# dkohlsdorf/audio_pattern_discovery

Measured on AMD Instinct MI355X. Metric: DTW cell-updates/sec (whole node), higher is better.
Workload: dtype f32

## Files before the change

audio_pattern_discovery_amd/csrc/dtw_systolic.h:

```cpp
#pragma once
#include <type_traits>

#ifndef APD_ABLATE
#define APD_ABLATE 0
#endif

#include "dtw_common.h"

namespace apd {

typedef float apd_f32x4 __attribute__((ext_vector_type(4)));
constexpr uint32_t kNoFrame = 0xFFFFFF00u;

template <int D>
__device__ __forceinline__ void load_frame(float (&dst)[D], __amdgpu_buffer_rsrc_t rsrc, uint32_t byte_off)
{
    constexpr int DP4 = (D + 3) / 4;
#pragma unroll
    for (int q = 0; q < DP4; ++q) {
        const apd_f32x4 t = __builtin_bit_cast(apd_f32x4, __builtin_amdgcn_raw_buffer_load_b128(rsrc, byte_off + 16u * q, 0, 0));
        if (4 * q + 0 < D) dst[4 * q + 0] = t.x;
        if (4 * q + 1 < D) dst[4 * q + 1] = t.y;
        if (4 * q + 2 < D) dst[4 * q + 2] = t.z;
        if (4 * q + 3 < D) dst[4 * q + 3] = t.w;
    }
}

template <int D>
__device__ __forceinline__ void load_frame_dwords(float (&dst)[D], __amdgpu_buffer_rsrc_t rsrc, uint32_t byte_off)
{
#pragma unroll
    for (int k = 0; k < D; ++k)
        dst[k] = __builtin_bit_cast(float, __builtin_amdgcn_raw_buffer_load_b32(rsrc, byte_off + 4u * k, 0, 0));
}

template <int D, int DN>
__device__ __forceinline__ float frame_dist(const float (&x)[DN], const float (&y)[DN])
{
    float t = x[0] - y[0];
    float acc = t * t;
#pragma unroll
    for (int k = 1; k < D; ++k) {
        t = x[k] - y[k];
        acc = __builtin_fmaf(t, t, acc);
    }
    if (APD_ABLATE & 1) return acc;
    return __builtin_amdgcn_sqrtf(acc);
}

template <int D, int DN>
__device__ __forceinline__ float frame_sq_strict(const float (&x)[DN], const float (&y)[DN])
{
    float t = x[0] - y[0];
    float acc = t * t;
#pragma unroll
    for (int k = 1; k < D; ++k) {
        t = x[k] - y[k];
        const float sq = t * t;
        acc = acc + sq;
    }
    return acc;
}
template <int D, int DN>
__device__ __forceinline__ float frame_dist_strict(const float (&x)[DN], const float (&y)[DN])
{
    return __builtin_sqrtf(frame_sq_strict<D, DN>(x, y));
}

template <int D>
__device__ __forceinline__ float frame_sq_expanded_pre(const float (&xm)[D + 1], const float (&y)[D + 1])
{
    float acc = xm[D] + y[D];
#pragma unroll
    for (int k = 0; k < D; ++k) acc = __builtin_fmaf(xm[k], y[k], acc);
    return acc;
}
template <int D>
__device__ __forceinline__ void prescale_row_piece(apd_f32x4 &v, int piece)
{
    const bool np = piece == D / 4;
    v.x = (np && D % 4 == 0) ? v.x : -2.0f * v.x;
    v.y = (np && D % 4 == 1) ? v.y : -2.0f * v.y;
    v.z = (np && D % 4 == 2) ? v.z : -2.0f * v.z;
    v.w = (np && D % 4 == 3) ? v.w : -2.0f * v.w;
}
template <int D>
__device__ __forceinline__ float frame_sq_exact_pre(const float (&xm)[D + 1], const float (&y)[D + 1])
{
    float t = __builtin_fmaf(-0.5f, xm[0], -y[0]);
    float acc = t * t;
#pragma unroll
    for (int k = 1; k < D; ++k) {
        t = __builtin_fmaf(-0.5f, xm[k], -y[k]);
        acc = __builtin_fmaf(t, t, acc);
    }
    return acc;
}
template <int C, int G, bool UNIFORM_PEN>
__device__ __forceinline__ void dp_rows_step(float (&prev1)[C], float (&prev2)[C], const float (&d)[C], const bool (&g1)[C],
                                             const bool (&g2)[C], float del, float ins, float mat, int gl)
{
    float left1 = group_from_lower_wrap<G>(prev1[C - 1], APD_INF, gl);
    float left2 = group_from_lower_wrap<G>(prev2[C - 1], APD_INF, gl);
    float upr1 = APD_INF, upr2 = APD_INF;
#pragma unroll
    for (int c = 0; c < C; ++c) {
        if (APD_ABLATE & 2) { prev1[c] += d[c]; prev2[c] -= d[c]; continue; }
        const float up1 = (c < C - 1) ? prev1[(c + 1) % C] : upr1;
        const float up2 = (c < C - 1) ? prev2[(c + 1) % C] : upr2;
        const float r1 = select_node<UNIFORM_PEN>(left1, up1, prev1[c], d[c], del, ins, mat, (APD_ABLATE & 16) ? false : g1[c]);
        const float r2 = select_node<UNIFORM_PEN>(up2, left2, prev2[c], d[c], del, ins, mat, (APD_ABLATE & 16) ? false : g2[c]);
        prev1[c] = r1; prev2[c] = r2;
        left1 = r1; left2 = r2;
        if (c == 0) {
            upr1 = group_from_upper_wrap<G>(r1, APD_INF, gl);
            upr2 = group_from_upper_wrap<G>(r2, APD_INF, gl);
        }
    }
}
template <int C>
__device__ __forceinline__ void slow_phase_captures(float (&prev1)[C], float (&prev2)[C], float &res1, float &res2, int tau, int gl,
                                                    int tau_cap, int cw, int cstar)
{
    if (tau == gl) {
#pragma unroll
        for (int c = 0; c < C; ++c) if (c == cw) { prev1[c] = 0.0f; prev2[c] = 0.0f; }
    }
    if (tau == tau_cap) {
#pragma unroll
        for (int c = 0; c < C; ++c) if (c == cstar) { res1 = prev1[c]; res2 = prev2[c]; }
    }
}
template <int D, int C, int G, bool UNIFORM_PEN, bool HYBRID>
__global__ __launch_bounds__(256) void dtw_fused_systolic(const AlignLaunch L)
{
    static_assert(C >= 2 && (64 % G) == 0, "bad geometry");
    if (L.d_nonfinite != nullptr && *L.d_nonfinite != 0u) return;
    constexpr int DN = D + 1;
    constexpr int DP = (DN + 3) & ~3;
    constexpr int PPW = 64 / G;
    constexpr int WPT = kSlotsPerTile / (4 * PPW);
    const int lane = threadIdx.x & 63;
    const int gl = lane % G;
    const uint32_t xcd = blockIdx.x & 7u, q = blockIdx.x >> 3;
    const uint32_t tile = (q / WPT) * 8u + xcd;
    const uint32_t slot = ((q % WPT) * 4u + (threadIdx.x >> 6)) * PPW + lane / G;
    const PairInfo P = decode_pair_rows_b(L, tile, slot);
    const bool special = P.valid && (P.n == 1 || P.m == 1);
    const bool sweep = P.valid && !special;
    if (__ballot(sweep) == 0ull) {
        if (special && gl == 0) { const float s = (P.n == 1 && P.m == 1) ? 0.0f : APD_INF; store_pair(L, tile, P, s, s); }
        return;
    }
    const int n = sweep ? P.n : 1, m = sweep ? P.m : 1, w = sweep ? P.w : 2;
    const __amdgpu_buffer_rsrc_t rsrc = __builtin_amdgcn_make_buffer_rsrc((void *)L.d_frames, 0, L.frames_bytes, 0x00020000);
    const uint32_t a_off = (uint32_t)(P.A - L.d_frames) * 4u, b_off = (uint32_t)(P.B - L.d_frames) * 4u;
    constexpr uint32_t FB = DP * 4u;
    float ins = L.band.ins, del = L.band.del, mat = L.band.mat;
    float tau_thr = L.tau, nmax_b = P.nmax_b;
    asm volatile("" : "+v"(ins), "+v"(del), "+v"(mat), "+v"(tau_thr), "+v"(nmax_b));
    constexpr int R = (G == 64) ? 128 : 64;
    constexpr int LPF = DP / 4;
    constexpr int FPF = 64 / LPF;
    constexpr int RS = DP + 4;
    constexpr int U_ROWS = ((C + 1) % 2 == 0) ? (C + 1) : 2 * (C + 1);
    __shared__ float xring_all[4][(R + U_ROWS) * RS];
    float *const xring = xring_all[threadIdx.x >> 6];
    const int lead = __builtin_ctzll(__ballot(sweep));
    const uint32_t a_off_w = __builtin_amdgcn_readlane(a_off, lead);
    const int n_w = __builtin_amdgcn_readlane(n, lead);
    const int u0 = C * gl;
    const int two_w = 2 * w;

    bool g1[C], g2[C];
#pragma unroll
    for (int c = 0; c < C; ++c) {
        const int u = u0 + c;
        g1[c] = u >= two_w;
        g2[c] = (u == 0) | (u > two_w);
    }
    const int cw = w - u0;
    const int ustar = sweep_result_offset(n, m, w);
    const int cstar = ustar - u0;
    const int tau_cap = (n - 1) + gl;

    int w_bound = w;
    asm volatile("" : "+v"(w_bound));
    int my_total = sweep ? sweep_steps_needed(n, m, w_bound, C) : 0;
    int my_min = sweep ? (n - 1) : 0x7fffffff;
    int total = 0, min_rows = 0x7fffffff;
#pragma unroll
    for (int g = 0; g < PPW; ++g) {
        total = max(total, __builtin_amdgcn_readlane(my_total, g * G));
        min_rows = min(min_rows, __builtin_amdgcn_readlane(my_min, g * G));
    }
    constexpr int S = C + 1;
    constexpr int U = (S % 2 == 0) ? S : 2 * S;
    static_assert(U == U_ROWS, "ring copy sized for another unroll");
    constexpr bool MASKED_FETCH = HYBRID && (G == 32 || G == 8) && !(APD_ABLATE & 512);
    const int total_r = ((total + U - 1) / U) * U;
    int a_steps = G;
    if (UNIFORM_PEN && !HYBRID) {
        int w_max = 0;
#pragma unroll
        for (int g = 0; g < PPW; ++g) w_max = max(w_max, __builtin_amdgcn_readlane(w, g * G));
        a_steps = max(G, w_max + 1);
    }
    const int a_end = min(((a_steps + U - 1) / U) * U, total_r);
    const int b_end = min(max((min_rows / U) * U, a_end), total_r);

    float prev1[C], prev2[C];
#pragma unroll
    for (int c = 0; c < C; ++c) { prev1[c] = APD_INF; prev2[c] = APD_INF; }
    float res1 = 0.0f, res2 = 0.0f;

    float yf[S][DN];
#pragma unroll
    for (int c = 0; c < C; ++c) {
        const int j = u0 - gl + c - w;
        const int idx = (j >= 1) ? (min(j, m) - 1) : (HYBRID ? m : m + 1);
        load_frame<DN>(yf[c], rsrc, b_off + (uint32_t)idx * FB);
    }
#pragma unroll
    for (int k = 0; k < DN; ++k) yf[C][k] = 0.0f;
    if (HYBRID && !MASKED_FETCH && !(APD_ABLATE & 8)) {
        const int jt = 1 + (C - 1) * G - w;
        const uint32_t yo = b_off + (uint32_t)((jt >= 1) ? (min(jt, m) - 1) : m) * FB;
        load_frame<DN>(yf[C], rsrc, gl == G - 1 ? yo : kNoFrame);
    }
    constexpr int NFILL = (U + FPF - 1) / FPF;
    const int fill_f = lane / LPF, fill_q = lane % LPF;
    auto fill_load = [&](int first_row, apd_f32x4 (&regs)[NFILL]) __attribute__((always_inline)) {
#pragma unroll
        for (int f = 0; f < NFILL; ++f) {
            const int fi = f * FPF + fill_f;
            const bool act = (fill_f < FPF) & (fi < U);
            const uint32_t off = a_off_w + (uint32_t)(min(first_row + fi, n_w) - 1) * FB + 16u * fill_q;
            regs[f] = __builtin_bit_cast(apd_f32x4, __builtin_amdgcn_raw_buffer_load_b128(rsrc, act ? off : kNoFrame, 0, 0));
        }
    };
    auto fill_store = [&](int first_row, const apd_f32x4 (&regs)[NFILL]) __attribute__((always_inline)) {
#pragma unroll
        for (int f = 0; f < NFILL; ++f) {
            const int fi = f * FPF + fill_f;
            if ((fill_f < FPF) & (fi < U)) {
                apd_f32x4 v = regs[f];
                if (HYBRID) prescale_row_piece<D>(v, fill_q);
                const int slot = (first_row + fi) & (R - 1);
                *reinterpret_cast<apd_f32x4 *>(&xring[slot * RS + 4 * fill_q]) = v;
                if (slot < U) *reinterpret_cast<apd_f32x4 *>(&xring[(slot + R) * RS + 4 * fill_q]) = v;
            }
        }
    };
    for (int e = lane; e < G * DP; e += 64) {
        const int slot = (-(e / DP)) & (R - 1);
        const float v = HYBRID ? ((e % DP) == D ? APD_INF : 0.0f) : -APD_INF;
        xring[slot * RS + (e % DP)] = v;
        if (slot < U) xring[(slot + R) * RS + (e % DP)] = v;
    }
    {
        apd_f32x4 regs[NFILL];
        fill_load(1, regs);
        fill_store(1, regs);
    }
    asm volatile("" ::: "memory");
    auto read_row = [&](float (&dst)[DN], int row) __attribute__((always_inline)) {
        const float *p = &xring[(row & (R - 1)) * RS];
#pragma unroll
        for (int q = 0; q < LPF; ++q) {
            const apd_f32x4 t = *reinterpret_cast<const apd_f32x4 *>(p + 4 * q);
            if (4 * q + 0 < DN) dst[4 * q + 0] = t.x;
            if (4 * q + 1 < DN) dst[4 * q + 1] = t.y;
            if (4 * q + 2 < DN) dst[4 * q + 2] = t.z;
            if (4 * q + 3 < DN) dst[4 * q + 3] = t.w;
        }
    };
    auto read_row_at = [&](float (&dst)[DN], const float *p) __attribute__((always_inline)) {
#pragma unroll
        for (int q = 0; q < LPF; ++q) {
            const apd_f32x4 t = *reinterpret_cast<const apd_f32x4 *>(p + 4 * q);
            if (4 * q + 0 < DN) dst[4 * q + 0] = t.x;
            if (4 * q + 1 < DN) dst[4 * q + 1] = t.y;
            if (4 * q + 2 < DN) dst[4 * q + 2] = t.z;
            if (4 * q + 3 < DN) dst[4 * q + 3] = t.w;
        }
    };
    constexpr int NX = HYBRID ? 1 : 2;
    float xs[NX][DN];
    read_row(xs[0], 0 - gl);
#pragma unroll
    for (int k = 0; k < DN; ++k) xs[NX - 1][k] = (NX == 1) ? xs[0][k] : 0.0f;
    constexpr bool PIPE = (APD_ABLATE & 32) != 0;
    float dn[C];
#pragma unroll
    for (int c = 0; c < C; ++c) dn[c] = (PIPE && !HYBRID && c < C - 1) ? frame_dist_strict<D, DN>(xs[0], yf[c]) : 0.0f;

    auto advance_window = [&](int q) __attribute__((always_inline)) {
        const int r = q % S, e = (r + C) % S;
#pragma unroll
        for (int k = 0; k < (HYBRID ? DN : D); ++k) {
            if (APD_ABLATE & 4) { yf[e][k] = yf[(r + 1) % S][k] + yf[e][k]; continue; }
            yf[e][k] = MASKED_FETCH ? dpp_move<(G == 8) ? 0x101 : 0x130>(yf[(r + 1) % S][k], yf[e][k])
                                    : group_from_upper<G>(yf[(r + 1) % S][k], yf[e][k], gl);
        }
    };
    auto macro_steps = [&](int tau_begin, int tau_end, auto slow_tag) __attribute__((always_inline)) {
        constexpr bool SLOW = decltype(slow_tag)::value;
        uint32_t yo_cur = kNoFrame, yo_cap = kNoFrame, yo_step = 0u;
        if (!SLOW && gl == G - 1) {
            yo_cap = b_off + (uint32_t)(m - 1) * FB;
            yo_cur = min(b_off + (uint32_t)(tau_begin + ((HYBRID && !MASKED_FETCH) ? 1 : 0) + (C - 1) * G - w) * FB, yo_cap);
            yo_step = FB;
        }
        auto fetch_column = [&](float (&dst)[DN], int t) __attribute__((always_inline)) {
            if (APD_ABLATE & 8) return;
            if (SLOW) {
                const int jt = t + 1 + (C - 1) * G - w;
                const uint32_t yo = b_off + (uint32_t)((jt >= 1) ? (min(jt, m) - 1) : (HYBRID ? m : m + 1)) * FB;
                load_frame<DN>(dst, rsrc, gl == G - 1 ? yo : kNoFrame);
            } else {
                load_frame<DN>(dst, rsrc, yo_cur);
                yo_cur = min(yo_cur + yo_step, yo_cap);
            }
        };
        for (int tau0 = tau_begin; tau0 < tau_end; tau0 += U) {
            apd_f32x4 fill_regs[NFILL];
            fill_load(tau0 + U + 1, fill_regs);
            const float *const xrows = &xring[((tau0 + 1 - gl) & (R - 1)) * RS];
#pragma unroll
            for (int q = 0; q < U; ++q) {
                const int tau = tau0 + q;
                const int r = q % S;
                const int xa = HYBRID ? 0 : (q & 1), xb = HYBRID ? 0 : (xa ^ 1);
                const int e = (r + C) % S;
                if (!HYBRID) {
                    fetch_column(yf[e], tau);
                    read_row_at(xs[xb], xrows + q * RS);
                }
                float d[C];
                if (HYBRID) {
#pragma unroll
                    for (int c = 0; c < C; ++c) {
                        d[c] = frame_sq_expanded_pre<D>(xs[xa], yf[(r + c) % S]);
                    }
                    float dmin = d[0];
#pragma unroll
                    for (int c = 1; c + 1 < C; c += 2) dmin = __builtin_fminf(__builtin_fminf(dmin, d[c]), d[c + 1]);
                    if (C % 2 == 0) dmin = __builtin_fminf(dmin, d[C - 1]);
                    const bool any = (APD_ABLATE & 128) ? false : dmin < (xs[xa][D] + nmax_b) * tau_thr;
                    advance_window(q);
                    if (MASKED_FETCH) {
                        if (gl == G - 1) fetch_column(yf[e], tau);
                    }
                    if (__builtin_expect(__ballot(any) != 0ull, 0)) {
                        float nx = xs[xa][D];
                        asm volatile("" : "+v"(nx));
#pragma unroll
                        for (int c = 0; c < C; ++c) {
                            const float sc = nx + yf[(r + c) % S][D];
                            const float ex = frame_sq_exact_pre<D>(xs[xa], yf[(r + c) % S]);
                            d[c] = (d[c] < sc * tau_thr) ? ex : d[c];
                        }
                    }
                    if (!MASKED_FETCH) fetch_column(yf[r], tau + 1);
#pragma unroll
                    for (int c = 0; c < C; ++c) d[c] = (APD_ABLATE & 1) ? d[c] : __builtin_amdgcn_sqrtf(d[c]);
                    read_row_at(xs[0], xrows + q * RS);
                } else if (UNIFORM_PEN && !SLOW && !PIPE) {
                    float d2[C];
#pragma unroll
                    for (int c = 0; c < C; ++c) d2[c] = frame_sq_strict<D, DN>(xs[xa], yf[(r + c) % S]);
                    float dmin = d2[0];
#pragma unroll
                    for (int c = 1; c + 1 < C; c += 2) dmin = __builtin_fminf(__builtin_fminf(dmin, d2[c]), d2[c + 1]);
                    if (C % 2 == 0) dmin = __builtin_fminf(dmin, d2[C - 1]);
                    if (__builtin_expect(__ballot(!(dmin >= 0x1p-96f)) != 0ull, 0)) {
#pragma unroll
                        for (int c = 0; c < C; ++c) d[c] = __builtin_sqrtf(d2[c]);
                    } else {
#pragma unroll
                        for (int c = 0; c < C; ++c) d[c] = sqrt_rn_finite(d2[c]);
                    }
                } else {
#pragma unroll
                    for (int c = 0; c < C; ++c)
                        d[c] = (UNIFORM_PEN && PIPE && c < C - 1) ? dn[c] : frame_dist_strict<D, DN>(xs[xa], yf[(r + c) % S]);
                    if (PIPE) {
#pragma unroll
                        for (int c = 0; c < C - 1; ++c) dn[c] = frame_dist_strict<D, DN>(xs[xb], yf[(r + 1 + c) % S]);
                    }
                }
                dp_rows_step<C, G, UNIFORM_PEN>(prev1, prev2, d, g1, g2, del, ins, mat, gl);
                if (SLOW) slow_phase_captures<C>(prev1, prev2, res1, res2, tau, gl, tau_cap, cw, cstar);
                if (!HYBRID) advance_window(q);
            }
            fill_store(tau0 + U + 1, fill_regs);
            asm volatile("" ::: "memory");
        }
    };
    macro_steps(0, a_end, std::true_type{});
    macro_steps(a_end, b_end, std::false_type{});
    macro_steps(b_end, total_r, std::true_type{});

    if (P.valid && gl == (sweep ? ustar / C : 0)) {
        if (sweep) {
            const float denom = (float)(n + m);
            store_pair_rows_b(L, tile, P, res1 / denom, res2 / denom);
        } else {
            const float s = (P.n == 1 && P.m == 1) ? 0.0f : APD_INF;
            store_pair(L, tile, P, s, s);
        }
    }
}

typedef float apd_f32x2 __attribute__((ext_vector_type(2)));
template <int DN>
__device__ __forceinline__ void read_frame_lds(float (&dst)[DN], const float *p)
{
    constexpr int FULL = DN / 4, TAIL = DN % 4;
#pragma unroll
    for (int k = 0; k < FULL; ++k) {
        const apd_f32x4 t = *reinterpret_cast<const apd_f32x4 *>(p + 4 * k);
        dst[4 * k + 0] = t.x; dst[4 * k + 1] = t.y; dst[4 * k + 2] = t.z; dst[4 * k + 3] = t.w;
    }
    if (TAIL >= 2) {
        const apd_f32x2 t = *reinterpret_cast<const apd_f32x2 *>(p + 4 * FULL);
        dst[4 * FULL + 0] = t.x; dst[4 * FULL + 1] = t.y;
    }
    if (TAIL == 1) dst[4 * FULL] = p[4 * FULL];
    if (TAIL == 3) dst[4 * FULL + 2] = p[4 * FULL + 2];
}

constexpr int shared_column_ring_floats(int rc, int u, int dp) { return (((rc + u) * dp + ((rc + u + 7) / 8) * 4) * 4 + 255) / 256 * 64; }

template <int D, int C, int G>
__global__ __launch_bounds__(256) void dtw_fused_systolic_shared(const AlignLaunch L)
{
    static_assert(C >= 2 && G == 16, "one ring per wavefront: four lane groups");
    if (L.d_nonfinite != nullptr && *L.d_nonfinite != 0u) return;
    constexpr int DN = D + 1;
    constexpr int DP = (DN + 3) & ~3;
    constexpr int PPW = 64 / G;
    constexpr int WPT = kSlotsPerTile / (4 * PPW);
    constexpr int S = C + 1;
    constexpr int U = shared_column_unroll(C);
    constexpr int RC = shared_column_ring_frames(G, C);
    constexpr int R = 64;
    constexpr int LPF = DP / 4;
    constexpr int FPF = 64 / LPF;
    constexpr int RS = DP + 4;
    constexpr uint32_t FB = DP * 4u;
    constexpr int XRING = (R + U) * RS;
    constexpr int CRING = shared_column_ring_floats(RC, U, DP);
    static_assert(FPF >= U && RC % 8 == 0, "one wave-wide load per fill");
    static_assert(RC >= (G - 1) * (C - 1) + 2 * U + (int)shared_column_slack(KernelGeom{KernelGeom::SharedColumns, G, C}),
                  "ring too short for the spread of w the tile plan admits");
    extern __shared__ __attribute__((aligned(16))) float apd_shared_lds[];
    const int lane = threadIdx.x & 63, wave = threadIdx.x >> 6;
    const int gl = lane % G;
    float *const xring = apd_shared_lds + wave * XRING;
    float *const crings = apd_shared_lds + 4 * XRING;
    int *const wg_words = reinterpret_cast<int *>(crings + PPW * CRING);
    const uint32_t xcd = blockIdx.x & 7u, q = blockIdx.x >> 3;
    const uint32_t tile = (q / WPT) * 8u + xcd;
    const uint32_t sub = q % WPT;
    const uint32_t slot = ((sub % 4u) * 4u + wave) * kTile + (sub / 4u) * 4u + lane / G;
    const PairInfo P = decode_pair_rows_b(L, tile, slot);
    const bool special = P.valid && (P.n == 1 || P.m == 1);
    const bool sweep = P.valid && !special;
    const int n = sweep ? P.n : 1, m = sweep ? P.m : 1, w = sweep ? P.w : 2;
    const int u0 = C * gl;
    const int two_w = 2 * w;
    int w_bound = w;
    asm volatile("" : "+v"(w_bound));
    int my_total = sweep ? sweep_steps_needed(n, m, w_bound, C) : 0;
    int my_min = sweep ? (n - 1) : 0x7fffffff;
    int my_w = sweep ? w : 0x7fffffff;
    int total = 0, min_rows = 0x7fffffff, w_lo = 0x7fffffff;
#pragma unroll
    for (int g = 0; g < PPW; ++g) {
        total = max(total, __builtin_amdgcn_readlane(my_total, g * G));
        min_rows = min(min_rows, __builtin_amdgcn_readlane(my_min, g * G));
        w_lo = min(w_lo, __builtin_amdgcn_readlane(my_w, g * G));
    }
    if (lane == 0) { wg_words[2 * wave] = total; wg_words[2 * wave + 1] = w_lo; }
    __syncthreads();
    total = 0; w_lo = 0x7fffffff;
#pragma unroll
    for (int k = 0; k < 4; ++k) { total = max(total, wg_words[2 * k]); w_lo = min(w_lo, wg_words[2 * k + 1]); }
    if (total == 0) {
        if (special && gl == 0) { const float s = (P.n == 1 && P.m == 1) ? 0.0f : APD_INF; store_pair(L, tile, P, s, s); }
        return;
    }
    const __amdgpu_buffer_rsrc_t rsrc = __builtin_amdgcn_make_buffer_rsrc((void *)L.d_frames, 0, L.frames_bytes, 0x00020000);
    const uint32_t a_off = (uint32_t)(P.A - L.d_frames) * 4u, b_off = (uint32_t)(P.B - L.d_frames) * 4u;
    float ins = L.band.ins, del = L.band.del, mat = L.band.mat;
    float tau_thr = L.tau, nmax_b = P.nmax_b;
    asm volatile("" : "+v"(ins), "+v"(del), "+v"(mat), "+v"(tau_thr), "+v"(nmax_b));
    const unsigned long long sweeping = __ballot(sweep);
    const int lead = sweeping ? __builtin_ctzll(sweeping) : 0;
    const uint32_t a_off_w = sweeping ? __builtin_amdgcn_readlane(a_off, lead) : 0u;
    const int n_w = sweeping ? __builtin_amdgcn_readlane(n, lead) : 1;
    uint32_t cb_off = 0u;
    int cm = 0;
    bool cvalid = false;
    {
        const uint4 t = L.d_tiles[tile];
        const uint32_t a = t.x * kTile + (sub / 4u) * 4u + wave;
        if (a < L.n_seq) {
            const uint32_t oa = L.d_seq_off[a];
            cm = (int)(L.d_seq_off[a + 1] - oa) - 2;
            cb_off = oa * L.dpad * 4u;
            cvalid = true;
        }
    }

    bool g1[C], g2[C];
#pragma unroll
    for (int c = 0; c < C; ++c) {
        const int u = u0 + c;
        g1[c] = u >= two_w;
        g2[c] = (u == 0) | (u > two_w);
    }
    const int cw = w - u0;
    const int ustar = sweep_result_offset(n, m, w);
    const int cstar = ustar - u0;
    const int tau_cap = (n - 1) + gl;
    const int total_r = ((total + U - 1) / U) * U;
    const int a_end = min(((G + U - 1) / U) * U, total_r);
    const int b_end = min(max((min_rows / U) * U, a_end), total_r);

    float prev1[C], prev2[C];
#pragma unroll
    for (int c = 0; c < C; ++c) { prev1[c] = APD_INF; prev2[c] = APD_INF; }
    float res1 = 0.0f, res2 = 0.0f;

    float yf[S][DN];
#pragma unroll
    for (int c = 0; c < C; ++c) {
        const int j = u0 - gl + c - w;
        const int idx = (j >= 1) ? (min(j, m) - 1) : m;
        load_frame<DN>(yf[c], rsrc, b_off + (uint32_t)idx * FB);
    }
#pragma unroll
    for (int k = 0; k < DN; ++k) yf[C][k] = 0.0f;

    constexpr int NFILL = (U + FPF - 1) / FPF;
    const int fill_f = lane / LPF, fill_q = lane % LPF;
    const bool fill_act = (fill_f < FPF) & (fill_f < U);
    auto fill_load = [&](int first_row, apd_f32x4 (&regs)[NFILL]) __attribute__((always_inline)) {
        const uint32_t off = a_off_w + (uint32_t)(min(first_row + fill_f, n_w) - 1) * FB + 16u * fill_q;
        regs[0] = __builtin_bit_cast(apd_f32x4, __builtin_amdgcn_raw_buffer_load_b128(rsrc, fill_act ? off : kNoFrame, 0, 0));
    };
    auto fill_store = [&](int first_row, const apd_f32x4 (&regs)[NFILL]) __attribute__((always_inline)) {
        if (fill_act) {
            apd_f32x4 v = regs[0];
            prescale_row_piece<D>(v, fill_q);
            const int rslot = (first_row + fill_f) & (R - 1);
            *reinterpret_cast<apd_f32x4 *>(&xring[rslot * RS + 4 * fill_q]) = v;
            if (rslot < U) *reinterpret_cast<apd_f32x4 *>(&xring[(rslot + R) * RS + 4 * fill_q]) = v;
        }
    };
    for (int e = lane; e < G * DP; e += 64) {
        const int rslot = (-(e / DP)) & (R - 1);
        const float v = (e % DP) == D ? APD_INF : 0.0f;
        xring[rslot * RS + (e % DP)] = v;
        if (rslot < U) xring[(rslot + R) * RS + (e % DP)] = v;
    }
    {
        apd_f32x4 regs[NFILL];
        fill_load(1, regs);
        fill_store(1, regs);
    }
    float *const cring_fill = crings + wave * CRING;
    const int col_hi0 = U + (C - 1) * G - w_lo;
    auto ring_slot = [](int j) { return (j + 64 * RC) % RC; };
    auto ring_at = [](auto *ring, uint32_t p) { return ring + p * DP + ((p >> 3) << 2); };
    auto col_load = [&](int j, bool act) __attribute__((always_inline)) {
        const int idx = (j >= 1) ? (min(j, cm) - 1) : cm;
        const uint32_t off = cb_off + (uint32_t)idx * FB + 16u * fill_q;
        return __builtin_bit_cast(apd_f32x4, __builtin_amdgcn_raw_buffer_load_b128(rsrc, (act & cvalid) ? off : kNoFrame, 0, 0));
    };
    for (int j0 = col_hi0 - RC + 1; j0 <= col_hi0; j0 += FPF) {
        const int j = j0 + fill_f;
        const bool act = (fill_f < FPF) & (j <= col_hi0);
        const apd_f32x4 v = col_load(j, act);
        const uint32_t ps = (uint32_t)ring_slot(j);
        if (act) *reinterpret_cast<apd_f32x4 *>(ring_at(cring_fill, ps) + 4 * fill_q) = v;
        if (act && ps < (uint32_t)U) *reinterpret_cast<apd_f32x4 *>(ring_at(cring_fill, ps + RC) + 4 * fill_q) = v;
    }
    uint32_t pf = (uint32_t)ring_slot(col_hi0 + 1 + fill_f);
    const float *const cring_read = crings + (lane / G) * CRING;
    uint32_t pr = (uint32_t)ring_slot(1 + (C - 1) * (gl + 1) - w);
    auto read_col = [&](float (&dst)[DN], const float *block_base, int q) __attribute__((always_inline)) {
        read_frame_lds<DN>(dst, block_base + q * DP + (((pr + (uint32_t)q) >> 3) << 2));
    };
    __syncthreads();
    auto read_row_at = [&](float (&dst)[DN], const float *p) __attribute__((always_inline)) { read_frame_lds<DN>(dst, p); };
    float xs[DN];
    read_row_at(xs, &xring[((0 - gl) & (R - 1)) * RS]);

    auto macro_steps = [&](int tau_begin, int tau_end, auto slow_tag) __attribute__((always_inline)) {
        constexpr bool SLOW = decltype(slow_tag)::value;
        for (int tau0 = tau_begin; tau0 < tau_end; tau0 += U) {
            apd_f32x4 fill_regs[NFILL];
            fill_load(tau0 + U + 1, fill_regs);
            const apd_f32x4 col_regs = col_load(tau0 + col_hi0 + 1 + fill_f, fill_act);
            const float *const xrows = &xring[((tau0 + 1 - gl) & (R - 1)) * RS];
            const float *const ycols = cring_read + pr * DP;
#pragma unroll
            for (int q = 0; q < U; ++q) {
                const int tau = tau0 + q;
                const int r = q % S;
                const int e = (r + C) % S;
                float d[C];
#pragma unroll
                for (int c = 0; c < C; ++c) d[c] = frame_sq_expanded_pre<D>(xs, yf[(r + c) % S]);
                float dmin = d[0];
#pragma unroll
                for (int c = 1; c + 1 < C; c += 2) dmin = __builtin_fminf(__builtin_fminf(dmin, d[c]), d[c + 1]);
                if (C % 2 == 0) dmin = __builtin_fminf(dmin, d[C - 1]);
                const bool any = dmin < (xs[D] + nmax_b) * tau_thr;
                read_col(yf[e], ycols, q);
                if (__builtin_expect(__ballot(any) != 0ull, 0)) {
                    float nx = xs[D];
                    asm volatile("" : "+v"(nx));
#pragma unroll
                    for (int c = 0; c < C; ++c) {
                        const float sc = nx + yf[(r + c) % S][D];
                        const float ex = frame_sq_exact_pre<D>(xs, yf[(r + c) % S]);
                        d[c] = (d[c] < sc * tau_thr) ? ex : d[c];
                    }
                }
#pragma unroll
                for (int c = 0; c < C; ++c) d[c] = __builtin_amdgcn_sqrtf(d[c]);
                read_row_at(xs, xrows + q * RS);
                dp_rows_step<C, G, true>(prev1, prev2, d, g1, g2, del, ins, mat, gl);
                if (SLOW) slow_phase_captures<C>(prev1, prev2, res1, res2, tau, gl, tau_cap, cw, cstar);
            }
            fill_store(tau0 + U + 1, fill_regs);
            if (fill_act) *reinterpret_cast<apd_f32x4 *>(ring_at(cring_fill, pf) + 4 * fill_q) = col_regs;
            if (fill_act && pf < (uint32_t)U) *reinterpret_cast<apd_f32x4 *>(ring_at(cring_fill, pf + RC) + 4 * fill_q) = col_regs;
            pf = min(pf + (uint32_t)U, pf + (uint32_t)U - (uint32_t)RC);
            pr = min(pr + (uint32_t)U, pr + (uint32_t)U - (uint32_t)RC);
            __syncthreads();
        }
    };
    macro_steps(0, a_end, std::true_type{});
    macro_steps(a_end, b_end, std::false_type{});
    macro_steps(b_end, total_r, std::true_type{});

    if (P.valid && gl == (sweep ? ustar / C : 0)) {
        if (sweep) {
            const float denom = (float)(n + m);
            store_pair_rows_b(L, tile, P, res1 / denom, res2 / denom);
        } else {
            const float s = (P.n == 1 && P.m == 1) ? 0.0f : APD_INF;
            store_pair(L, tile, P, s, s);
        }
    }
}

template <int D, int C, int G>
constexpr size_t shared_columns_lds_bytes()
{
    constexpr int DP = (D + 1 + 3) & ~3, U = shared_column_unroll(C), RC = shared_column_ring_frames(G, C);
    constexpr int XRING = (64 + U) * (DP + 4), CRING = shared_column_ring_floats(RC, U, DP);
    return (size_t)(4 * XRING + (64 / G) * CRING + 8) * sizeof(float);
}
template <int D, int C, int G>
static hipError_t launch_shared_columns_kernel(const AlignLaunch &L, hipStream_t stream)
{
    constexpr int WPT = kSlotsPerTile / (4 * (64 / G));
    constexpr size_t lds = shared_columns_lds_bytes<D, C, G>();
    static_assert(lds <= 80 * 1024, "two workgroups per CU");
    static bool granted[64] = {};
    int dev = 0;
    if (hipError_t e = hipGetDevice(&dev); e != hipSuccess) return e;
    if (dev < 0 || dev >= 64 || !granted[dev]) {
        const hipError_t e = hipFuncSetAttribute(reinterpret_cast<const void *>(dtw_fused_systolic_shared<D, C, G>),
                                                 hipFuncAttributeMaxDynamicSharedMemorySize, (int)lds);
        if (e != hipSuccess) return e;
        if (dev >= 0 && dev < 64) granted[dev] = true;
    }
    const uint32_t tiles8 = (L.n_tiles + 7u) / 8u * 8u;
    hipLaunchKernelGGL((dtw_fused_systolic_shared<D, C, G>), dim3(tiles8 * WPT), dim3(256), lds, stream, L);
    return hipSuccess;
}

template <int D, int C, int G, bool UNIFORM_PEN, bool HYBRID>
static void launch_systolic_kernel(const AlignLaunch &L, hipStream_t stream)
{
    constexpr int PPW = 64 / G;
    constexpr int WPT = kSlotsPerTile / (4 * PPW);
    const uint32_t tiles8 = (L.n_tiles + 7u) / 8u * 8u;
    hipLaunchKernelGGL((dtw_fused_systolic<D, C, G, UNIFORM_PEN, HYBRID>), dim3(tiles8 * WPT), dim3(256), 0, stream, L);
}

#ifdef APD_SYSTOLIC_STRICT_UNIT
template <int D>
bool launch_systolic_strict(const AlignLaunch &L, KernelGeom g, hipStream_t stream)
{
#define APD_CASE(GG, CC) if constexpr (geom_instantiated(KernelGeom{KernelGeom::Systolic, GG, CC}, D)) { \
        if (g == KernelGeom{KernelGeom::Systolic, GG, CC}) { launch_systolic_kernel<D, CC, GG, true, false>(L, stream); return true; } }
    APD_SYSTOLIC_GEOMS(APD_CASE)
#undef APD_CASE
    return false;
}
#else
template <int D>
bool launch_systolic(const AlignLaunch &L, KernelGeom g, hipStream_t stream)
{
    const bool unit = L.band.ins == 1.0f && L.band.del == 1.0f && L.band.mat == 1.0f;
    if (g.family == KernelGeom::SharedColumns) {
        if (!(unit && L.hybrid)) return false;
#define APD_CASE(GG, CC) if constexpr (geom_instantiated(KernelGeom{KernelGeom::SharedColumns, GG, CC}, D)) { \
        if (g == KernelGeom{KernelGeom::SharedColumns, GG, CC}) return launch_shared_columns_kernel<D, CC, GG>(L, stream) == hipSuccess; }
        APD_SHARED_COLUMN_GEOMS(APD_CASE)
#undef APD_CASE
        return false;
    }
    if (unit && !L.hybrid) return launch_systolic_strict<D>(L, g, stream);
#define APD_CASE(GG, CC) if constexpr (geom_instantiated(KernelGeom{KernelGeom::Systolic, GG, CC}, D)) { \
        if (g == KernelGeom{KernelGeom::Systolic, GG, CC}) { \
            if (!unit) launch_systolic_kernel<D, CC, GG, false, false>(L, stream); else launch_systolic_kernel<D, CC, GG, true, true>(L, stream); \
            return true; } }
    APD_SYSTOLIC_GEOMS(APD_CASE)
#undef APD_CASE
    return false;
}
#endif

}
```

Baseline: 3199 billion.

## Interleave next-row LDS reads with distance FMAs and strength-reduce buffer offsets

The inner distance loop now reads the next row frame from LDS piece by piece, interleaved with the FMA chunks of the current distance computation, and issues the column LDS read earlier. This is meant to hide LDS latency behind ALU work. Global prefetch offsets for the row and column fill are now kept as running, clamped byte offsets instead of being recomputed each step, and LDS addresses are handled as raw 32-bit values. The rare exact-distance path must reload the current row frame from the ring, which adds LDS traffic when it triggers, and the extra live values raise register pressure.

```diff
diff --git a/audio_pattern_discovery_amd/csrc/dtw_systolic.h b/audio_pattern_discovery_amd/csrc/dtw_systolic.h
--- a/audio_pattern_discovery_amd/csrc/dtw_systolic.h
+++ b/audio_pattern_discovery_amd/csrc/dtw_systolic.h
@@ -415,13 +415,13 @@
 
 typedef float apd_f32x2 __attribute__((ext_vector_type(2)));
 template <int DN>
-__device__ __forceinline__ void read_frame_lds(float (&dst)[DN], const float *p)
+__device__ __forceinline__ void read_frame_piece_lds(float (&dst)[DN], const float *p, int piece)
 {
     constexpr int FULL = DN / 4, TAIL = DN % 4;
-#pragma unroll
-    for (int k = 0; k < FULL; ++k) {
-        const apd_f32x4 t = *reinterpret_cast<const apd_f32x4 *>(p + 4 * k);
-        dst[4 * k + 0] = t.x; dst[4 * k + 1] = t.y; dst[4 * k + 2] = t.z; dst[4 * k + 3] = t.w;
+    if (piece < FULL) {
+        const apd_f32x4 t = *reinterpret_cast<const apd_f32x4 *>(p + 4 * piece);
+        dst[4 * piece + 0] = t.x; dst[4 * piece + 1] = t.y; dst[4 * piece + 2] = t.z; dst[4 * piece + 3] = t.w;
+        return;
     }
     if (TAIL >= 2) {
         const apd_f32x2 t = *reinterpret_cast<const apd_f32x2 *>(p + 4 * FULL);
@@ -430,6 +430,16 @@
     if (TAIL == 1) dst[4 * FULL] = p[4 * FULL];
     if (TAIL == 3) dst[4 * FULL + 2] = p[4 * FULL + 2];
 }
+template <int DN>
+__device__ __forceinline__ void read_frame_lds(float (&dst)[DN], const float *p)
+{
+#pragma unroll
+    for (int piece = 0; piece < (DN + 3) / 4; ++piece) read_frame_piece_lds<DN>(dst, p, piece);
+}
+
+typedef __attribute__((address_space(3))) const char apd_lds_cchar;
+__device__ __forceinline__ uint32_t lds_address(const void *p) { return (uint32_t)(uintptr_t)(apd_lds_cchar *)p; }
+__device__ __forceinline__ const float *lds_floats_at(uint32_t a) { return (const float *)(apd_lds_cchar *)(uintptr_t)a; }
 
 constexpr int shared_column_ring_floats(int rc, int u, int dp) { return (((rc + u) * dp + ((rc + u + 7) / 8) * 4) * 4 + 255) / 256 * 64; }
 
@@ -592,49 +602,79 @@
     uint32_t pf = (uint32_t)ring_slot(col_hi0 + 1 + fill_f);
     const float *const cring_read = crings + (lane / G) * CRING;
     uint32_t pr = (uint32_t)ring_slot(1 + (C - 1) * (gl + 1) - w);
-    auto read_col = [&](float (&dst)[DN], const float *block_base, int q) __attribute__((always_inline)) {
-        read_frame_lds<DN>(dst, block_base + q * DP + (((pr + (uint32_t)q) >> 3) << 2));
+    const uint32_t ro_step = fill_act ? (uint32_t)U * FB : 0u;
+    const uint32_t ro_cap = fill_act ? a_off_w + (uint32_t)(n_w - 1) * FB + 16u * fill_q : kNoFrame;
+    uint32_t ro_cur = fill_act ? min(a_off_w + (uint32_t)(U + fill_f) * FB + 16u * fill_q, ro_cap) : kNoFrame;
+    const bool col_act = fill_act & cvalid;
+    const uint32_t co_step = col_act ? (uint32_t)U * FB : 0u;
+    const uint32_t co_cap = col_act ? cb_off + (uint32_t)(cm - 1) * FB + 16u * fill_q : kNoFrame;
+    uint32_t co_cur = col_act ? min(cb_off + (uint32_t)(col_hi0 + fill_f) * FB + 16u * fill_q, co_cap) : kNoFrame;
+    const uint32_t cring_read_b = lds_address(cring_read);
+    uint32_t col_base = 0u;
+    auto read_col = [&](float (&dst)[DN], int q) __attribute__((always_inline)) {
+        const uint32_t b = (col_base + 2u * (uint32_t)q) & ~15u;
+        read_frame_lds<DN>(dst, lds_floats_at(b) + q * DP);
     };
     __syncthreads();
-    auto read_row_at = [&](float (&dst)[DN], const float *p) __attribute__((always_inline)) { read_frame_lds<DN>(dst, p); };
     float xs[DN];
-    read_row_at(xs, &xring[((0 - gl) & (R - 1)) * RS]);
+    read_frame_lds<DN>(xs, &xring[((0 - gl) & (R - 1)) * RS]);
+    static_assert(R > U + G - 1, "a macro-step's row frame must survive in the ring until the block's fill_store");
 
     auto macro_steps = [&](int tau_begin, int tau_end, auto slow_tag) __attribute__((always_inline)) {
         constexpr bool SLOW = decltype(slow_tag)::value;
         for (int tau0 = tau_begin; tau0 < tau_end; tau0 += U) {
             apd_f32x4 fill_regs[NFILL];
-            fill_load(tau0 + U + 1, fill_regs);
-            const apd_f32x4 col_regs = col_load(tau0 + col_hi0 + 1 + fill_f, fill_act);
-            const float *const xrows = &xring[((tau0 + 1 - gl) & (R - 1)) * RS];
-            const float *const ycols = cring_read + pr * DP;
+            fill_regs[0] = __builtin_bit_cast(apd_f32x4, __builtin_amdgcn_raw_buffer_load_b128(rsrc, ro_cur, 0, 0));
+            const apd_f32x4 col_regs = __builtin_bit_cast(apd_f32x4, __builtin_amdgcn_raw_buffer_load_b128(rsrc, co_cur, 0, 0));
+            ro_cur = min(ro_cur + ro_step, ro_cap);
+            co_cur = min(co_cur + co_step, co_cap);
+            uint32_t xrows_b = lds_address(xring) + (uint32_t)(((tau0 + 1 - gl) & (R - 1)) * RS) * 4u;
+            col_base = cring_read_b + __umul24(pr, FB + 2u);
+            asm volatile("" : "+v"(xrows_b), "+v"(col_base));
+            const float *const xrows = lds_floats_at(xrows_b);
 #pragma unroll
             for (int q = 0; q < U; ++q) {
                 const int tau = tau0 + q;
                 const int r = q % S;
                 const int e = (r + C) % S;
                 float d[C];
-#pragma unroll
-                for (int c = 0; c < C; ++c) d[c] = frame_sq_expanded_pre<D>(xs, yf[(r + c) % S]);
+                read_col(yf[e], q);
+                const float *const xnext = xrows + q * RS;
+                const float thr = (xs[D] + nmax_b) * tau_thr;
+#pragma unroll
+                for (int c = 0; c < C; ++c) d[c] = xs[D] + yf[(r + c) % S][D];
+#pragma unroll
+                for (int piece = 0; piece < LPF; ++piece) {
+#pragma unroll
+                    for (int k = 4 * piece; k < 4 * piece + 4 && k < D; ++k)
+#pragma unroll
+                        for (int c = 0; c < C; ++c) d[c] = __builtin_fmaf(xs[k], yf[(r + c) % S][k], d[c]);
+#pragma unroll
+                    for (int c = 0; c < C; ++c) asm volatile("" : "+v"(d[c]) : : "memory");
+                    read_frame_piece_lds<DN>(xs, xnext, piece);
+                }
                 float dmin = d[0];
 #pragma unroll
                 for (int c = 1; c + 1 < C; c += 2) dmin = __builtin_fminf(__builtin_fminf(dmin, d[c]), d[c + 1]);
                 if (C % 2 == 0) dmin = __builtin_fminf(dmin, d[C - 1]);
-                const bool any = dmin < (xs[D] + nmax_b) * tau_thr;
-                read_col(yf[e], ycols, q);
+                const bool any = dmin < thr;
+                asm volatile("" : : : "memory");
                 if (__builtin_expect(__ballot(any) != 0ull, 0)) {
-                    float nx = xs[D];
+                    float xc[DN];
+                    read_frame_lds<DN>(xc, &xring[((tau - gl) & (R - 1)) * RS]);
+                    float nx = xc[D];
                     asm volatile("" : "+v"(nx));
 #pragma unroll
                     for (int c = 0; c < C; ++c) {
                         const float sc = nx + yf[(r + c) % S][D];
-                        const float ex = frame_sq_exact_pre<D>(xs, yf[(r + c) % S]);
+                        const float ex = frame_sq_exact_pre<D>(xc, yf[(r + c) % S]);
                         d[c] = (d[c] < sc * tau_thr) ? ex : d[c];
                     }
+                    asm volatile("" : : : "memory");
+                    read_frame_lds<DN>(xs, xnext);
                 }
 #pragma unroll
                 for (int c = 0; c < C; ++c) d[c] = __builtin_amdgcn_sqrtf(d[c]);
-                read_row_at(xs, xrows + q * RS);
                 dp_rows_step<C, G, true>(prev1, prev2, d, g1, g2, del, ins, mat, gl);
                 if (SLOW) slow_phase_captures<C>(prev1, prev2, res1, res2, tau, gl, tau_cap, cw, cstar);
             }
```

Result: faster. 3326 billion, median of 6 (+4.0%).
